# Dane-ME/keypoint-detection

Measured on AMD Instinct MI355X. Metric: images/sec @ 256x192 COCO-17 (MultiPersonKeypointModel.forward, given boxes), higher is better.
Workload: dtype fp32; 1 GPU; C2: batch 64/GPU, 256x192x3, 1 box/img, heatmap head + soft-argmax decode; model=MultiPersonKeypointModel (MobileNetV3-Small+FPN, HeatmapHead), global_batch=64, height=256, width=192, persons=1, precision=split, parallelism=dp1, streams_per_gpu=1, gather=False, gather_pipelined=False

## Files before the change

### include/kpd.h

```cpp
#ifndef KPD_H_
#define KPD_H_

#include <stddef.h>
#include <stdint.h>

#ifdef __cplusplus
extern "C" {
#endif

#define KPD_OK 0
#define KPD_EINVAL (-1)
#define KPD_EHIP (-2)
#define KPD_ESTATE (-3)

#define KPD_PRECISION_FP32 0
#define KPD_PRECISION_MIXED 1
#define KPD_PRECISION_SPLIT 2

typedef struct kpd_plan kpd_plan;

const char* kpd_last_error(void);
const char* kpd_version(void);

int kpd_plan_create(int device, int in_channels, kpd_plan** out);
// ... 115 lines not shown
                              void* stream);

#define KPD_COORD_SMOOTH_L1 0
#define KPD_COORD_MSE 1
#define KPD_COORD_HUBER 2
int kpd_coord_loss(const float* heat, const float* gt, const float* vis, int planes, int H, int W, float temperature,
                   int loss_type, float pixel_weight_scale, float distance_threshold, float* coords, float* loss,
                   float* grad, void* stream);

int kpd_softargmax_backward(const float* heat, const float* grad_coords, int planes, int H, int W, float temperature,
                            float* grad_heat, void* stream);

int kpd_plan_set_streams(kpd_plan* plan, int n);

int kpd_plan_set_graphs(kpd_plan* plan, int enable);

int kpd_bench_conv16(int split, int N, int H, int W, int cin, int cout, int dbg, int iters, float* ms);

#define KPD_BUILD_DIAG 1
int kpd_build_flags(void);

int kpd_fpn0x_class_table(int* cls_ng, int* cls_g, int* cls_woff, int* blocks);


int kpd_heatmap_head(kpd_plan* plan, const float* x, int R, int H, int W, int parts, float* heat, float* ch_w,
                     float* sp_w, void* stream);

int kpd_keypoint_head(kpd_plan* plan, const float* x, int R, int H, int W, float* keypoints, float* visibility,
                      void* stream);

int kpd_backbone(kpd_plan* plan, const float* image, int B, int C, int H, int W, float* out0, float* out1,
                 float* out2, float* out3, void* stream);

int kpd_backbone_body(kpd_plan* plan, const float* image, int B, int C, int H, int W, float* feat0, float* feat1,
                      float* feat2, float* feat3, void* stream);

int kpd_backbone_fpn(kpd_plan* plan, const float* feat0, const float* feat1, const float* feat2, const float* feat3,
                     int B, const int* sizes, float* out0, float* out1, float* out2, float* out3, void* stream);

int kpd_roi_features(kpd_plan* plan, const float* image, int B, int C, int H, int W, const float* boxes, int P,
                     const int32_t* rows, int n, float* out, void* stream);

int kpd_channel_attention(kpd_plan* plan, const float* x, int B, int C, int H, int W, float* scores, int32_t* topk,
                          int k, float* selected, void* stream);

#define KPD_DECODE_ARGMAX 0
// ... 48 lines not shown
```

### keypoint-detection_amd/csrc/conv_glds.hip

```cpp
#include <algorithm>
#include <type_traits>

#include "kpd_common.h"
#include "kpd_kernels.h"
#include "conv_epilogue.h"
#include "kpd_dma.h"

namespace {

typedef _Float16 f16x8 __attribute__((ext_vector_type(8)));
typedef __attribute__((address_space(3))) void lds_void;

constexpr int BM = 256, NT = 512, ROWB = 128;
constexpr unsigned OOB = 0x80000000u;

__device__ __forceinline__ void stamp16(unsigned long long* st, int i, unsigned long long v = 0, int row = -1) {
  if (st && threadIdx.x == 0)
    st[(size_t)(row < 0 ? blockIdx.x : row) * 8 + i] = v ? v : __builtin_amdgcn_s_memrealtime();
}

__device__ __forceinline__ float dpp_xor1(float x) {
  return __int_as_float(__builtin_amdgcn_mov_dpp(__float_as_int(x), 0xB1, 0xF, 0xF, true));
}
__device__ __forceinline__ float dpp_xor2(float x) {
// ... 519 lines not shown
    }
    s_fp[u] = make_int2(x0 | (x1 << 16), y0 | (y1 << 16));
  }
  __syncthreads();
  const int f_tsel = (lchunk >> 1) & 1;
  const unsigned f_byte = (unsigned)((lchunk >> 2) * 32 + (lchunk & 1) * 16);
  const int co_b = wave * (BN / 8) + lrow;

  int cls = 0, n = 0, jt = 0, ca = 0, cb = 0, q0 = 0, NG = 1, NL = 0, KT = 0, ld = 0;
  constexpr int FSH = 22;
  unsigned f_off[A_LD], l_off = 0;
  const float inv_rw = 1.f / (float)rw;
  auto rows = [&](int L, unsigned* fo, unsigned& lo) {
    const int c = L & 15, nj = L >> 4, nn = nj / p.tpc, j = nj - nn * p.tpc;
    const int a_ = c >> 2, b_ = c & 3, qb = j * BM;
    lo = (unsigned)((nn * RG + qb + wave * 32 + lrow) * 512);
#pragma unroll
    for (int i = 0; i < A_LD; ++i) {
      const int q = qb + wave * 32 + i * 8 + lrow;
      const int Y = (int)(((float)q + 0.5f) * inv_rw), X = q - Y * rw, y = 4 * Y + a_, x = 4 * X + b_;
      const unsigned fl = (y > 0 ? 1u : 0u) | (y + 1 < Hf ? 2u : 0u) | (x > 0 ? 4u : 0u) | (x + 1 < Wf ? 8u : 0u) |
                          (Y > 0 ? 16u : 0u) | (Y + 1 < rh ? 32u : 0u) | (X > 0 ? 64u : 0u) |
                          (X + 1 < rw ? 128u : 0u) | (q < RG ? 256u : 0u);
      fo[i] = (unsigned)((nn * Hf + y) * Wf + x) | fl << FSH;
    }
  };
  auto need = [](int dy, int dx, int sh) {
    return ((dy < 0 ? 1u : 0u) | (dy > 0 ? 2u : 0u) | (dx < 0 ? 4u : 0u) | (dx > 0 ? 8u : 0u)) << sh | 256u;
  };
  auto setup = [&](int L) {
    cls = L & 15;
    const int nj = L >> 4;
    n = nj / p.tpc;
    jt = nj - n * p.tpc;
    ca = cls >> 2;
    cb = cls & 3;
    q0 = jt * BM;
    NG = s_ng[cls];
    NL = (kFpn0xSecondMask >> cls) & 1u ? 0 : 4 * NG;
    KT = NL + KT0;
    ld = 0;
  };
  auto issue_tap0 = [&](int stage, int k, const unsigned* fo) {
    const unsigned so = stage * STAGE;
    const int t = 2 * k + f_tsel;
    const int dy = t / 3 - 1, dx = t % 3 - 1;
    const int delta = (dy * Wf + dx) * 64 + (int)f_byte;
    const unsigned nd = t < 9 ? need(dy, dx, 0) : ~0u;
#pragma unroll
    for (int i = 0; i < A_LD; ++i) {
      const unsigned voff = ((fo[i] >> FSH) & nd) == nd ? ((fo[i] << (32 - FSH)) >> (32 - FSH - 6)) + delta : OOB;
      glds16(rf, a_dst + so + i * 8 * ROWB, voff, 0);
    }
#pragma unroll
    for (int i = 0; i < B_LD; ++i)
      glds16(rw0, b_dst + so + i * 8 * ROWB, (unsigned)(((co_b + i * 8) * KT0 + k) * ROWB + lchunk * 16), 0);
  };
  auto issue_at = [&](int stage, int k, int c, int ng, int nl, const unsigned* fo, unsigned lo) {
    const unsigned so = stage * STAGE;
    if (k >= nl) {
      issue_tap0(stage, k - nl, fo);
    } else {
      const int g = k >> 2, kc = k & 3;
      const int gg = s_g[c * 4 + g], oy = gg / 3 - 1, ox = gg % 3 - 1;
      const int delta = (oy * rw + ox) * 512 + kc * 128 + lchunk * 16;
      const unsigned nd = need(oy, ox, 4);
#pragma unroll
      for (int i = 0; i < A_LD; ++i) {
        const unsigned voff = ((fo[i] >> FSH) & nd) == nd ? lo + i * 8 * 512 + delta : OOB;
        glds16(rl, a_dst + so + i * 8 * ROWB, voff, 0);
      }
      const int wbase = s_woff[c] * 2;
#pragma unroll
      for (int i = 0; i < B_LD; ++i)
        glds16(rwe, b_dst + so + i * 8 * ROWB,
               (unsigned)(wbase + (((co_b + i * 8) * ng + g) * 4 + kc) * ROWB + lchunk * 16), 0);
    }
  };
  auto issue = [&](int stage) {
    issue_at(stage, ld, cls, NG, NL, f_off, l_off);
    ++ld;
  };

  f32x4 acc[FM][FN];
// ... 170 lines not shown
        sts[(WAVES_M + wm) * BN + col + r16] = mx;
      }
    }
    __builtin_amdgcn_s_waitcnt(0xC07F);
    __builtin_amdgcn_s_barrier();
    asm volatile("" ::: "memory");
    stamp16(p.stamps, 7, 0, L);
    {
      float v = 0.f;
      if (tid < 2 * BN) {
        const int c = tid & (BN - 1), mxs = tid >= BN;
        v = sts[mxs * WAVES_M * BN + c];
#pragma unroll
        for (int w = 1; w < WAVES_M; ++w) {
          const float u = sts[(mxs * WAVES_M + w) * BN + c];
          v = mxs ? fmaxf(v, u) : v + u;
        }
      }
      const unsigned so = (unsigned)(((e_n * 16 + e_cls) * p.tpc + e_jt) * 2 * BN) * 4u;
      __builtin_amdgcn_raw_buffer_store_b32(__builtin_bit_cast(unsigned, v), rst, tid < 2 * BN ? so + tid * 4 : OOB, 0, 0);
    }
    stamp16(p.stamps, 3, 0, L);
    const int src4 = ((lane & 0x30) | ((lane & 3) << 2) | ((lane >> 2) & 3)) * 4;
    const int2 fp = s_fp[e_n];
    const int fx0 = fp.x & 0xFFFF, fx1 = fp.x >> 16, fy0 = fp.y & 0xFFFF, fy1 = fp.y >> 16;
#pragma unroll
    for (int i = 0; i < FM; ++i)
#pragma unroll
      for (int e = 0; e < 4; ++e) {
        f32x4 v = f32x4{acc[i][0][e], acc[i][1][e], acc[i][2][e], acc[i][3][e]};
        quad_transpose(v, t4);
        f32x4 w;
#pragma unroll
        for (int k = 0; k < 4; ++k) w[k] = __int_as_float(__builtin_amdgcn_ds_bpermute(src4, __float_as_int(v[k])));
        const int q = e_q0 + wm * WM + i * 16 + g * 4 + e;
        const int Y = (int)(((float)q + 0.5f) * inv_rw), X = q - Y * rw;
        const unsigned o =
            (unsigned)((((e_n * Hf + 4 * Y + e_ca) * Wf + 4 * X + e_cb) * BN + wn * 64 + r16 * 4) * 4);
        const int py = 4 * Y + e_ca, px = 4 * X + e_cb;
        const bool keep = q < RG && py >= fy0 && py <= fy1 && px >= fx0 && px <= fx1;
        const unsigned so = keep && (DBG != 4 || (i | e) == 0) ? o : OOB;
        if (p.out_nt) __builtin_amdgcn_raw_buffer_store_b128(__builtin_bit_cast(u32x4, w), rout, so, 0, 2);
        else __builtin_amdgcn_raw_buffer_store_b128(__builtin_bit_cast(u32x4, w), rout, so, 0, 0);
      }
    L = Lnext;
  }
}

// ... 2 lines not shown
                                                         int w_expE, _Float16* __restrict__ out) {
  const int G = cin == 16 ? 16 : 32, c8n = cin / 8;
  const long i = (long)blockIdx.x * blockDim.x + threadIdx.x;
  if (i >= (long)N * hw * c8n) return;
  const long px = i / c8n;
  const int c = (int)(i - px * c8n) * 8, n = (int)(px / hw);
  int a_f, a_l, P;
  fpn0x_exps(sc[(size_t)n * kAmaxStride], sc[(size_t)(N + n) * kAmaxStride], w_exp0, w_expE, &a_f, &a_l, &P);
  const float s = ldexpf(1.f, which ? a_l : a_f);
  const float4 u = *reinterpret_cast<const float4*>(in + px * cin + c);
  const float4 v = *reinterpret_cast<const float4*>(in + px * cin + c + 4);
  const float x[8] = {u.x, u.y, u.z, u.w, v.x, v.y, v.z, v.w};
  typedef _Float16 f16x8v __attribute__((ext_vector_type(8)));
  f16x8v hi, lo;
#pragma unroll
  for (int e = 0; e < 8; ++e) {
    const float xs = x[e] * s;
    hi[e] = (_Float16)xs;
    lo[e] = (_Float16)(xs - (float)hi[e]);
  }
  _Float16* o = out + px * 2 * cin + (c / G) * 2 * G + c % G;
  *reinterpret_cast<f16x8v*>(o) = hi;
  *reinterpret_cast<f16x8v*>(o + G) = lo;
}

constexpr int HP = kHmPitch, HPP = kHmRoiPos;
constexpr int HMS = 56;
constexpr int AWIN = 384;
template <int BMH>
constexpr int hm_awin() { return BMH + 128 <= AWIN ? AWIN : BMH + 128; }
template <int BMH>
constexpr int hm_epi_parts() { return BMH > 256 ? 2 : 1; }
template <int CIN, bool SPLIT>
constexpr int hm_nab() { return (CIN > 0 && (SPLIT ? CIN * 4 : CIN * 2) == 128) ? 1 : 2; }
template <int BMH>
constexpr int kh_epi_parts() { return BMH > 128 ? 2 : 1; }
template <int BN, int BMH>
constexpr int kh_epi_bytes() { return BMH / kh_epi_parts<BMH>() * ((BN + 4) + 68) * 4; }
template <int BN, int SB, int BMH, bool SPLIT, int TPS, int NW, int MODE, int NAB = 2>
constexpr int hmconv_lds_bytes() {
  constexpr int EMODE = MODE >= 0 ? MODE : (BN == 64 ? 1 : 0);
  constexpr int RING = NAB * hm_awin<BMH>() * ROWB + SB * BN * ROWB * TPS;
  constexpr int EPI = EMODE == 2 ? (BN == 128 ? kh_epi_bytes<BN, BMH>() : 0)
                      : EMODE != 0 && EMODE != 3 ? 0 : epi_lds_bytes<BMH / hm_epi_parts<BMH>(), 128, NW * 64>();
  return RING > EPI ? RING : EPI;
}
// ... 1162 lines not shown
  b.stagger = stagger ? 1 : 0;
  static const int out_nt = kpd_diag_env("KPD_FPN0X_NT") ? atoi(kpd_diag_env("KPD_FPN0X_NT")) : 1;
  b.out_nt = out_nt;
  b.spn = spn;
#if KPD_DIAG
  if (dbg == 1) hipLaunchKernelGGL(fpn0x_kernel<1>, dim3((unsigned)grid), dim3(NT), 0, st, b);
  else if (dbg == 2) hipLaunchKernelGGL(fpn0x_kernel<2>, dim3((unsigned)grid), dim3(NT), 0, st, b);
  else if (dbg == 4) hipLaunchKernelGGL(fpn0x_kernel<4>, dim3((unsigned)grid), dim3(NT), 0, st, b);
  else
#endif
  hipLaunchKernelGGL(fpn0x_kernel<0>, dim3((unsigned)grid), dim3(NT), 0, st, b);
  return hipGetLastError();
}

hipError_t launch_split_rows(const float* in, int N, long hw, int cin, const float* sc, int which, int w_exp0,
                             int w_expE, void* out, hipStream_t st) {
  if (cin != 16 && cin % 32 != 0) return hipErrorInvalidValue;
  const long n = (long)N * hw * (cin / 8);
  hipLaunchKernelGGL(split_rows_kernel, dim3((unsigned)((n + 255) / 256)), dim3(256), 0, st, in, N, hw, cin, sc,
                     which, w_exp0, w_expE, static_cast<_Float16*>(out));
  return hipGetLastError();
}

template <int DBG>
static hipError_t bench_launch(const Conv16Args& a, int split, hipStream_t st) {
  if constexpr (DBG == 0) return launch_conv16(a, split, split ? 0 : 1, st);
  dim3 grid(((a.M + BM - 1) / BM) * (a.cout_p / 128));
  if (split) hipLaunchKernelGGL((conv16_kernel<true, float, 3, 128, 3, true, DBG>), grid, dim3(NT), 0, st, a);
  else hipLaunchKernelGGL((conv16_kernel<false, __bf16, 3, 128, 3, true, DBG>), grid, dim3(NT), 0, st, a);
  return hipGetLastError();
}

extern "C" int kpd_bench_conv16(int split, int N, int H, int W, int cin, int cout, int dbg, int iters, float* ms) {
  if (N <= 0 || H <= 0 || W <= 0 || cin % 64 || cout % 128 || iters <= 0 || !ms) return -1;
  if (split && (cin != 128 || cout != 128)) return -1;
  Conv16Args a{};
  const long M = (long)N * H * W;
  const int cin_e = split ? 2 * cin : cin;
  const long in_b = M * cin_e * 2, w_b = (long)cout * 9 * cin_e * 2, out_b = M * cout * 4;
  if (in_b > kMaxDesc) return -1;
  void *in = nullptr, *wt = nullptr, *out = nullptr, *bias = nullptr, *stats = nullptr;
  const bool with_stats = split && ((long)H * W) % BM == 0;
  hipEvent_t e0 = nullptr, e1 = nullptr;
  int rc = -2;
  if (hipMalloc(&in, in_b) != hipSuccess || hipMalloc(&wt, w_b) != hipSuccess || hipMalloc(&out, out_b) != hipSuccess ||
      hipMalloc(&bias, cout * 4) != hipSuccess ||
// ... 44 lines not shown
```

### keypoint-detection_amd/csrc/kpd_common.h

```cpp
#pragma once
#include <hip/hip_runtime.h>
#include <hip/hip_bf16.h>
#include <stdint.h>
#include <stdlib.h>

#ifndef KPD_DIAG
#define KPD_DIAG 0
#endif
static inline const char* kpd_diag_env(const char* name) {
#if KPD_DIAG
  return getenv(name);
#else
  (void)name;
  return nullptr;
#endif
}

typedef float f32x4 __attribute__((ext_vector_type(4)));
typedef __bf16 bf16x8 __attribute__((ext_vector_type(8)));
typedef __bf16 bf16x4 __attribute__((ext_vector_type(4)));
typedef _Float16 f16x4 __attribute__((ext_vector_type(4)));

__device__ __forceinline__ float kpd_div6(float x) {
  constexpr float r6 = 1.f / 6.f;
// ... 40 lines not shown
__device__ __forceinline__ int slot_pos(int s) { return (-1 - s) & 0xFFFF; }
__device__ __forceinline__ bool slot_dummy(int s) { return ((-1 - s) >> 16) & 1; }

__device__ __forceinline__ void amax_publish_img(float* slots, int n, float v) {
  if (v > 0.f) atomicMax(reinterpret_cast<unsigned int*>(slots + (size_t)n * kAmaxStride), __float_as_uint(v));
}

__device__ __forceinline__ int split_exp_of(float amax) {
  const float u = amax * 1.0078125f;
  if (!(u > 0.f)) return 100;
  if (!(u < INFINITY)) return -100;
  int e;
  frexpf(u, &e);
  return min(max(14 - e, -100), 100);
}
__device__ __forceinline__ void fpn0x_exps(float f, float l, int w_exp0, int w_expE, int* a_f, int* a_l, int* P) {
  int pp = min(split_exp_of(f) + w_exp0, split_exp_of(l) + w_expE);
  pp = min(max(pp, -120), 120);
  *P = pp;
  *a_f = pp - w_exp0;
  *a_l = pp - w_expE;
}

#define KPD_CHECK_LAUNCH() (hipGetLastError())
```

### keypoint-detection_amd/csrc/kpd_kernels.h

```cpp
#pragma once
#include <hip/hip_runtime.h>
#include <stdint.h>
#include <vector>

struct ConvArgs {
  const void* in;
  const void* wt;
  const float* bias;
  void* out;
  const float* res;
  const float* a_scale;
  float* stats;
  int N, H, W;
  int cin_p, cout_p;
  int in_cstride, out_cstride;
  int rh, rw;
  int act;
  int M;
  int tiles_per_img;
  float* amax;
  const float* post_scale;
  const float* post_shift;
  int act2, act3;
  int in_bytes, wt_bytes;
// ... 74 lines not shown
  const void* l_split;
  const void* w0;
  const void* weff;
  int cls_woff[16];
  int cls_ng[16];
  int cls_g[16][kFpn0xMaxGroups];
  const float* bias;
  float* out;
  float* stats;
  const float* sc;
  int sc_n;
  int N, Hf, Wf, rh, rw, tpc, w_exp0, w_expE;
  int f_bytes, l_bytes, w0_bytes, weff_bytes;
  int stagger;
  int out_nt;
  int spn;
  unsigned long long* stamps;
  const float* fp_boxes;
  int fp_NB, fp_P;
};
hipError_t launch_fpn0x(const Fpn0xArgs& a, hipStream_t st);
hipError_t launch_split_rows(const float* in, int N, long hw, int cin, const float* sc, int which, int w_exp0,
                             int w_expE, void* out, hipStream_t st);
int conv16_tile_m();

enum ConvDType : int { CONV_F32 = 0, CONV_BF16_OUT_BF16 = 1, CONV_BF16_OUT_F32 = 2 };

int conv_tile_m();
hipError_t launch_conv(const ConvArgs& a, ConvDType dt, int ks, hipStream_t st);

hipError_t launch_stem(const float* img, int N, int Cin, int H, int W, const float* w, const float* b,
                       float* out, int Ho, int Wo, float* amax, hipStream_t st);
hipError_t launch_dwconv(const float* in, const float* w, const float* b, float* out, int N, int H, int W,
                         int Cp, int Ho, int Wo, int k, int s, int act, hipStream_t st);
hipError_t launch_se(const float* x, int N, int HW, int C, int Cp, const float* w1, const float* b1,
                     const float* w2, const float* b2, int sq, float* scale, hipStream_t st,
                     const float* pooled = nullptr);
struct FirArgs {
  const float* x;
  int Hi, Wi, cin_p;
  const float *we, *be;
  const float *wd, *bd;
  const float *wp, *bp;
  int act_e, act_d, Ep, cout_p;
  float* out;
  int Ho, Wo, res;
// ... 265 lines not shown
```

### keypoint-detection_amd/csrc/kpd_pack.hip

```cpp
#include "kpd_plan_int.h"

namespace {

int se_squeeze(int c) {
  const int v = c / 4;
  int n = std::max(8, (int)(v + 4) / 8 * 8);
  if (n < 0.9 * v) n += 8;
  return n;
}

uint16_t f2bf(float f) {
  uint32_t u;
  std::memcpy(&u, &f, 4);
  if ((u & 0x7fffffffu) > 0x7f800000u) return (uint16_t)((u >> 16) | 0x40);
  u += 0x7fffu + ((u >> 16) & 1u);
  return (uint16_t)(u >> 16);
}

const HostT* get(kpd_plan* p, const std::string& name, std::string& missing) {
  auto it = p->t.find(name);
  if (it == p->t.end()) {
    missing += name + " ";
    return nullptr;
  }
// ... 314 lines not shown
                     hE.data() + p->fpn0x.cls_woff[cls]);
  }
  if (int rc = upload(p, h0, &p->fpn0x.w0)) return rc;
  if (int rc = upload(p, hE, &p->fpn0x.weff)) return rc;
  p->fpn0x.w0_bytes = (int)(h0.size() * 2);
  p->fpn0x.weff_bytes = (int)(hE.size() * 2);
  p->fpn0x.w_exp0 = e0;
  p->fpn0x.w_expE = eE;
  return KPD_OK;
}

}

extern "C" {

int kpd_fpn0x_class_table(int* cls_ng, int* cls_g, int* cls_woff, int* blocks) {
  if (!cls_ng || !cls_g || !cls_woff || !blocks) return fail(KPD_EINVAL, "NULL output");
  const int nb = fpn0x_class_table(cls_ng, reinterpret_cast<int(*)[kFpn0xMaxGroups]>(cls_g), cls_woff);
  if (nb < 0) return fail(KPD_ESTATE, "fpn0x: inconsistent class table");
  *blocks = nb;
  return KPD_OK;
}

int kpd_plan_finalize(kpd_plan* p, int precision) {
  if (!p) return fail(KPD_EINVAL, "null plan");
  if (precision != KPD_PRECISION_FP32 && precision != KPD_PRECISION_MIXED && precision != KPD_PRECISION_SPLIT)
    return fail(KPD_EINVAL, "unknown precision");
  HIP_TRY(hipSetDevice(p->device));
  for (void* a : p->allocs) (void)hipFree(a);
  p->allocs.clear();
  p->fpn0x.w0 = p->fpn0x.weff = nullptr;
  p->stamps = nullptr;
  p->pd = DevConv();
  p->anchors = nullptr;
  p->hm1 = DevConv();
  p->hm2 = DevConv();
  p->hm3 = DevConv();
  for (auto& c : p->fpn_lv) c = DevConv();
  p->kh_ds1 = DevConv();
  p->kh_ds2 = DevConv();
  for (auto& k : p->kh_s) k = KhSplit();
  p->kh_split = false;
  p->has_kh = false;
  for (int k = 0; k <= kpd_plan::kMaxSub; ++k) {
    if (p->ws[k]) { (void)hipFree(p->ws[k]); p->ws[k] = nullptr; p->ws_bytes[k] = 0; }
    p->have_work[k] = false;
// ... 213 lines not shown
```

### keypoint-detection_amd/csrc/kpd_plan.hip

```cpp
#include "kpd_plan_int.h"

namespace {
thread_local std::string g_err;
}

int fail(int code, const std::string& msg) {
  g_err = msg;
  return code;
}

int kpd_fail_einval(const char* msg) { return fail(KPD_EINVAL, msg); }
int kpd_fail_hip(hipError_t e, const char* where) {
  return fail(KPD_EHIP, std::string(where) + ": " + hipGetErrorString(e));
}

thread_local KpdPathLog* g_kpd_path = nullptr;

namespace {
struct PathRow { const char* name; unsigned sites; };
const PathRow kPathRows[KP_COUNT] = {
#define KPD_PATH_ROW(id, name, sites) {name, sites},
    KPD_PATH_TOKENS(KPD_PATH_ROW)
#undef KPD_PATH_ROW
};
// ... 775 lines not shown
  lc.c1 = pad16(kFpnIn[1]); lc.c2 = pad16(kFpnIn[2]); lc.c3 = pad16(kFpnIn[3]);
  lc.c1r = kFpnIn[1]; lc.c2r = kFpnIn[2]; lc.c3r = kFpnIn[3];
  lc.S1 = p->lat_S[1]; lc.S2 = p->lat_S[2]; lc.S3 = p->lat_S[3];
  lc.w_exp0 = p->fpn0x.w_exp0; lc.w_expE = p->fpn0x.w_expE;
  lc.h1 = d.h[3]; lc.w1 = d.w[3]; lc.h2 = d.h[8]; lc.w2 = d.w[8]; lc.h3 = d.h[11]; lc.w3 = d.w[11];
  lc.lat1 = w.lat[1];
  lc.lat1_split = ps.lin ? reinterpret_cast<_Float16*>(reinterpret_cast<char*>(w.lat[0]) + (size_t)B * d.h[0] * d.w[0] * 64)
                         : nullptr;
  lc.amax = ps.lin ? w.sc : nullptr;
  static const bool no_chain_t0 = kpd_diag_env("KPD_NO_CHAIN_TAP0") != nullptr;
  if (ps.lin && !no_chain_t0) {
    lc.t0 = taps[0];
    lc.t0_split = reinterpret_cast<_Float16*>(w.lat[0]);
    lc.P0 = d.h[0] * d.w[0];
  }
  lc.stamps = ps.take_stamps("stamps_latchain_0", (size_t)8 * ((B + 7) / 8 * 8));
}

static int lateral0_split_rows(Pass& ps, const float* const taps[4], bool chain, bool chain_t0) {
  kpd_plan* p = ps.p; Work& w = *ps.w; const Dims& d = ps.d;
  char* base = reinterpret_cast<char*>(w.lat[0]);
  if (!chain || !chain_t0) {
    kpd_path(KP_SPLIT_ROWS);
    HIP_TRY(launch_split_rows(taps[0], d.B, (long)d.h[0] * d.w[0], 16, w.sc, 0, p->fpn0x.w_exp0, p->fpn0x.w_expE, base,
                              ps.st));
  }
  if (!chain) {
    kpd_path_at(KP_LAT, 1);
    kpd_path(KP_SPLIT_ROWS);
    HIP_TRY(launch_split_rows(w.lat[1], d.B, (long)d.h[3] * d.w[3], 128, w.sc, 1, p->fpn0x.w_exp0, p->fpn0x.w_expE,
                              base + (size_t)d.B * d.h[0] * d.w[0] * 64, ps.st));
  }
  return KPD_OK;
}

static int stage_laterals(Pass& ps, const float* const taps[4], bool keep_all) {
  kpd_plan* p = ps.p; Work& w = *ps.w; const Dims& d = ps.d;
  const int B = d.B;
  const int lh[4] = {d.h[0], d.h[3], d.h[8], d.h[11]}, lw[4] = {d.w[0], d.w[3], d.w[8], d.w[11]};
  const Stage stage(p, "fpn_lateral", ps.st);
  static const bool no_chain = kpd_diag_env("KPD_NO_LAT_CHAIN") != nullptr;
  LatChainArgs lc{};
  lateral_chain_fill(ps, taps, lc);
  const bool chain = !no_chain && !keep_all && !p->lat[1].bf16 && !p->lat[2].bf16 && !p->lat[3].bf16 &&
                     p->lat[1].cin_p == lc.c1 && p->lat[2].cin_p == lc.c2 && p->lat[3].cin_p == lc.c3 &&
                     p->lat[1].cout_p == 128 && p->lat[2].cout_p == 128 && p->lat[3].cout_p == 128 &&
                     lateral_chain_ok(lc);
  kpd_path(chain ? KP_LAT_CHAIN : KP_LAT_PER_LEVEL);
// ... 65 lines not shown
}

static int stage_topk(Pass& ps, const FwdArgs& a) {
  kpd_plan* p = ps.p; Work& w = *ps.w; const Dims& d = ps.d;
  const int B = d.B, HWf = d.Hf * d.Wf;
  const Stage stage(p, "topk", ps.st);
  if (!d.fused_stats) {
    kpd_path(KP_CHANNEL_STATS);
    HIP_TRY(launch_channel_stats(w.feat, B, HWf, 128, d.tiles, w.stats, ps.st));
  }
  const bool slot_in_topk = a.slot_in_topk();
  if (slot_in_topk) kpd_path(KP_TOPK_SLOTMAP);
  HIP_TRY(launch_topk(w.stats, B, d.tiles, HWf, p->ca_w0, p->ca_b0, p->ca_w2, p->ca_b2, w.topk, w.scores, ps.st,
                      slot_in_topk ? a.boxes : nullptr, a.P, slot_in_topk ? w.slot : nullptr, w.imax,
                      ps.lin ? w.sc : nullptr, B));
  if (ps.lin) w.sc_dirty = false;
  return KPD_OK;
}

static int publish_backbone(Pass& ps, const FwdArgs& a, const float* const taps[4]) {
  Work& w = *ps.w; const Dims& d = ps.d;
  const size_t B = d.B;
  if (a.topk_out) HIP_TRY(hipMemcpyAsync(a.topk_out, w.topk, sizeof(int32_t) * B * 64, hipMemcpyDeviceToDevice, ps.st));
  if (!level0_footprint(ps, a)) ps.dbg["feat0"] = {w.feat, sizeof(float) * B * d.Hf * d.Wf * 128};
  ps.dbg["scores"] = {w.scores, sizeof(float) * B * 128};
  ps.dbg["tap0"] = {taps[0], sizeof(float) * B * d.h[0] * d.w[0] * 16};
  ps.dbg["tap1"] = {taps[1], sizeof(float) * B * d.h[3] * d.w[3] * pad16(24)};
  ps.dbg["tap2"] = {taps[2], sizeof(float) * B * d.h[8] * d.w[8] * pad16(48)};
  ps.dbg["tap3"] = {taps[3], sizeof(float) * B * d.h[11] * d.w[11] * 576};
  if (ps.debug) ps.p->debug = ps.dbg;
  return KPD_OK;
}

static int stage_detect(Pass& ps, const FwdArgs& a) {
  kpd_plan* p = ps.p; Work& w = *ps.w; const Dims& d = ps.d;
  const int B = d.B;
  const Stage sg(p, "person_detect", ps.st);
  static const bool pd_unfused = kpd_diag_env("KPD_PD_UNFUSED") != nullptr;
  if (!pd_unfused && p->pd.cin == 128 && p->pd.cin_p == 128 && p->pd.cout_p == 48 && !p->pd.bf16 &&
      person_detect_fits(d.Wf)) {
    kpd_path(KP_PD_FUSED);
    HIP_TRY(launch_person_detect(w.feat, B, d.Hf, d.Wf, static_cast<const float*>(p->pd.w), p->pd.b, p->anchors, a.H,
                                 a.W, p->det_conf, w.pd_boxes, w.pd_scores, ps.st));
  } else {
    kpd_path(KP_PD_UNFUSED);
    HIP_TRY(launch_adaptive_pool56(w.feat, B, d.Hf, d.Wf, 128, w.pd_pool, ps.st));
    kpd_path_at(KP_PD);
// ... 707 lines not shown
```

### keypoint-detection_amd/csrc/lateral_chain.hip

```cpp
#include <algorithm>

#include "kpd_common.h"
#include "kpd_kernels.h"

namespace {

constexpr int LG = 16;

__device__ __forceinline__ int up_index(int y, int H, int h) {
  return H == h ? y : min((int)floorf((float)y * ((float)h / (float)H)), h - 1);
}

__device__ __forceinline__ void stamp(unsigned long long* st, int i) {
  if (st && threadIdx.x == 0)
    st[((size_t)blockIdx.y * gridDim.x + blockIdx.x) * 8 + i] = __builtin_amdgcn_s_memrealtime();
}

__device__ __forceinline__ f32x4 mfma_k16(const float4 a, const float4 b, f32x4 acc) {
  acc = __builtin_amdgcn_mfma_f32_16x16x4f32(a.x, b.x, acc, 0, 0, 0);
  acc = __builtin_amdgcn_mfma_f32_16x16x4f32(a.y, b.y, acc, 0, 0, 0);
  acc = __builtin_amdgcn_mfma_f32_16x16x4f32(a.z, b.z, acc, 0, 0, 0);
  return __builtin_amdgcn_mfma_f32_16x16x4f32(a.w, b.w, acc, 0, 0, 0);
}

// ... 186 lines not shown
          const int y = pp / p.w1, x = pp - y * p.w1;
          const int sy = up_index(y, p.h1, p.h2), sx = up_index(x, p.w1, p.w2);
          const float v = acc[e] + l2[(sy * p.w2 + sx) * LG + r16];
          if constexpr (SPLIT) {
            const float xs = v * s_l;
            const _Float16 hi = (_Float16)xs;
            tsc[(4 * g + e) * 32 + r16] = hi;
            tsc[(4 * g + e) * 32 + 16 + r16] = (_Float16)(xs - (float)hi);
          } else {
            out[(size_t)pp * 128] = v;
          }
        }
        if constexpr (SPLIT) {
          const int q = lane >> 2, pp = t * 16 + q;
          const uint4 v = *reinterpret_cast<const uint4*>(tsc + q * 32 + part * 8);
          if (pp < P1) *reinterpret_cast<uint4*>(outs + (size_t)pp * 256) = v;
        }
      }
    }
  }
  stamp(p.stamps, 4);
  if constexpr (SPLIT) {
    if (p.t0) {
      const int P0 = p.P0, n8 = P0 * 2, per = (n8 + 7) / 8, i0 = cg * per, i1 = min(i0 + per, n8);
      const float* src = p.t0 + (size_t)b * P0 * 16;
      _Float16* dst = p.t0_split + (size_t)b * P0 * 32;
      typedef _Float16 f16x8v __attribute__((ext_vector_type(8)));
      for (int j0 = i0 + tid; j0 < i1; j0 += 4 * NW * 64) {
        float4 u[4][2];
#pragma unroll
        for (int v = 0; v < 4; ++v) {
          const int j = min(j0 + v * NW * 64, i1 - 1), px = j >> 1, c = (j & 1) * 8;
          u[v][0] = *reinterpret_cast<const float4*>(src + (size_t)px * 16 + c);
          u[v][1] = *reinterpret_cast<const float4*>(src + (size_t)px * 16 + c + 4);
        }
#pragma unroll
        for (int v = 0; v < 4; ++v) {
          const int j = j0 + v * NW * 64, px = j >> 1, c = (j & 1) * 8;
          if (j >= i1) continue;
          const float x[8] = {u[v][0].x, u[v][0].y, u[v][0].z, u[v][0].w, u[v][1].x, u[v][1].y, u[v][1].z, u[v][1].w};
          f16x8v hi, lo;
#pragma unroll
          for (int e = 0; e < 8; ++e) {
            const float xs = x[e] * s_f;
            hi[e] = (_Float16)xs;
            lo[e] = (_Float16)(xs - (float)hi[e]);
          }
          _Float16* o = dst + (size_t)px * 32 + c;
          *reinterpret_cast<f16x8v*>(o) = hi;
          *reinterpret_cast<f16x8v*>(o + 16) = lo;
        }
      }
    }
  }
  stamp(p.stamps, 5);
}

}

size_t lateral_chain_lds_bytes(const LatChainArgs& a) {
  const size_t P2 = (size_t)a.h2 * a.w2, P3 = (size_t)a.h3 * a.w3;
  return (P3 * LG + std::max(P2, NW * P3) * LG + 4 * NW) * sizeof(float) + (size_t)NW * 16 * 2 * LG * 2;
}

bool lateral_chain_ok(const LatChainArgs& a) {
  return a.c1 == 32 && a.c2 == 48 && a.c3 == 576 && a.h1 > 0 && a.w1 > 0 && a.h2 > 0 && a.w2 > 0 && a.h3 > 0 &&
         a.w3 > 0 && a.h3 * a.w3 <= 16 * 8 && lateral_chain_lds_bytes(a) <= 80 * 1024 &&
         (!a.lat1_split || a.amax);
}

hipError_t launch_lateral_chain(const LatChainArgs& a, int B, hipStream_t st) {
  if (B <= 0) return hipSuccess;
  if (!lateral_chain_ok(a)) return hipErrorInvalidValue;
  LatChainArgs q = a;
  q.n = B;
  const dim3 grid((unsigned)((B + 7) / 8 * 8), 128 / LG), block(NW * 64);
  const size_t lds = lateral_chain_lds_bytes(a);
  const bool small = a.h3 * a.w3 <= 16 * 3;
  static const bool noreuse = kpd_diag_env("KPD_LC_NOREUSE") != nullptr;
  const bool reuse = !noreuse && (long)a.h1 * a.w1 <= 6 * NW * 16;
  if (a.lat1_split && small && reuse) {
    kpd_path(KP_LC_SPLIT_SMALL_REUSE);
    hipLaunchKernelGGL((lateral_chain_kernel<2, 3, 36, 3, 6, true, true>), grid, block, lds, st, q);
  } else if (a.lat1_split && reuse) {
    kpd_path(KP_LC_SPLIT_BIG_REUSE);
    hipLaunchKernelGGL((lateral_chain_kernel<2, 3, 36, 8, 6, true, true>), grid, block, lds, st, q);
  } else if (a.lat1_split) {
    kpd_path(small ? KP_LC_SPLIT_SMALL : KP_LC_SPLIT_BIG);
    if (small) hipLaunchKernelGGL((lateral_chain_kernel<2, 3, 36, 3, 6, true>), grid, block, lds, st, q);
    else hipLaunchKernelGGL((lateral_chain_kernel<2, 3, 36, 8, 6, true>), grid, block, lds, st, q);
  } else {
// ... 7 lines not shown
```

### keypoint-detection_amd/dll/_native.py

```python
from __future__ import annotations

import ctypes
import os
from pathlib import Path
from typing import List, Optional

import torch

_LIB_PATH = Path(__file__).resolve().parent / "_lib" / "libkpd.so"
_lib: Optional[ctypes.CDLL] = None

KPD_PRECISION_FP32 = 0
KPD_PRECISION_MIXED = 1
KPD_PRECISION_SPLIT = 2
PRECISIONS = {"fp32": KPD_PRECISION_FP32, "split": KPD_PRECISION_SPLIT, "mixed": KPD_PRECISION_MIXED,
              "bf16": KPD_PRECISION_MIXED}

EXPORTS = ("kpd_last_error", "kpd_version", "kpd_plan_create", "kpd_plan_set_tensor",
           "kpd_plan_finalize", "kpd_plan_destroy", "kpd_forward", "kpd_debug_copy", "kpd_nms",
           "kpd_plan_timing", "kpd_plan_timing_stage", "kpd_plan_timing_query", "kpd_plan_set_detector",
           "kpd_bench_conv16", "kpd_build_flags", "kpd_fpn0x_class_table",
           "kpd_plan_set_streams", "kpd_preprocess", "kpd_target_heatmaps", "kpd_keypoint_metrics",
           "kpd_heatmap_head", "kpd_keypoint_head", "kpd_backbone", "kpd_channel_attention", "kpd_decode_heatmaps",
           "kpd_roi_align", "kpd_conv1x1", "kpd_adaptive_heatmap_loss", "kpd_conv3x3_forward",
           "kpd_conv3x3_backward", "kpd_conv3x3_forward_prec", "kpd_conv3x3_backward_prec", "kpd_plan_set_graphs", "kpd_backbone_body", "kpd_backbone_fpn",
           "kpd_plan_path_log", "kpd_plan_path_query", "kpd_preprocess_batch", "kpd_draw_poses",
           "kpd_oks_match", "kpd_pose_nms", "kpd_flip_merge", "kpd_augment_batch", "kpd_bn_train_forward",
           "kpd_bn_train_backward", "kpd_roi_targets", "kpd_roi_features", "kpd_detector_features",
           "kpd_detector_targets", "kpd_detector_loss", "kpd_coord_loss", "kpd_softargmax_backward")
PRE_BATCH_CHUNK = 32
DRAW_BOXES, DRAW_LIMBS, DRAW_JOINTS, DRAW_HEAT = 1, 2, 4, 8
DRAW_CHUNK = 32
DRAW_TILE_W = 64
DRAW_TILE_H = 16
DRAW_MAX_SIDE = 16384
DRAW_MAX_WIDTH = 512
DRAW_MAX_HEAT = 1024
OKS_MAX_K = 32
OKS_MAX_T = 16
OKS_MAX_D = 64
OKS_MAX_G = 64
POSE_NMS_MAX_D = 64
POSE_NMS_MAX_K = 32
POSE_NMS_HARD, POSE_NMS_SOFT, POSE_NMS_SOFT_LINEAR = 0, 1, 2
# ... 60 lines not shown
    lib.kpd_plan_path_query.argtypes = [c_void_p, c_char_p, ctypes.c_size_t, ctypes.POINTER(ctypes.c_size_t)]
    lib.kpd_target_heatmaps.argtypes = [c_void_p, c_int, c_int, c_int, ctypes.c_double, c_void_p, c_void_p]
    lib.kpd_keypoint_metrics.argtypes = [c_void_p, c_void_p, c_void_p, ctypes.c_long, ctypes.POINTER(ctypes.c_float),
                                         c_int, c_void_p, c_void_p]
    lib.kpd_preprocess_batch.argtypes = [ctypes.POINTER(c_void_p), ctypes.POINTER(c_int), ctypes.POINTER(c_int),
                                         ctypes.POINTER(c_int), c_int, c_int, c_int, ctypes.c_float, c_int, c_int,
                                         c_int, c_int, ctypes.POINTER(ctypes.c_float),
                                         ctypes.POINTER(ctypes.c_float), c_void_p, c_void_p]
    u8p = ctypes.POINTER(ctypes.c_uint8)
    lib.kpd_draw_poses.argtypes = [ctypes.POINTER(c_void_p), ctypes.POINTER(c_int), ctypes.POINTER(c_int),
                                   ctypes.POINTER(c_int), c_int, c_void_p, c_void_p, c_void_p, c_void_p,
                                   c_int, c_int, c_int, c_int, ctypes.POINTER(c_int), c_int, u8p, u8p, u8p,
                                   c_int, c_int, c_int, c_int, c_int, c_int, c_int, c_void_p]
    lib.kpd_oks_match.argtypes = [c_void_p] * 8 + [ctypes.POINTER(ctypes.c_float)] * 2 + [c_int] * 6 + \
        [c_void_p] * 8
    lib.kpd_pose_nms.argtypes = [c_void_p] * 5 + [ctypes.POINTER(ctypes.c_float)] + [c_int] * 4 + \
        [ctypes.c_float] * 3 + [c_int] + [c_void_p] * 6
    lib.kpd_flip_merge.argtypes = [c_void_p] * 3 + [ctypes.POINTER(ctypes.c_int32)] + [c_int] * 5 + [c_void_p] * 5
    i32p = ctypes.POINTER(ctypes.c_int32)
    lib.kpd_augment_batch.argtypes = [ctypes.POINTER(c_void_p)] + [ctypes.POINTER(c_int)] * 3 + \
        [ctypes.POINTER(c_void_p), c_int, c_int, i32p, ctypes.POINTER(ctypes.c_double), ctypes.POINTER(c_int),
         i32p, i32p, u8p, i32p, c_void_p, c_void_p, c_void_p, c_int, c_int, c_void_p, c_void_p, c_void_p, c_void_p]
    lib.kpd_fpn0x_class_table.argtypes = [ctypes.POINTER(c_int)] * 4
    lib.kpd_nms.argtypes = [c_void_p, c_void_p, c_int, ctypes.c_float, c_int, c_void_p, c_void_p, c_void_p]
    c_float = ctypes.c_float
    lib.kpd_heatmap_head.argtypes = [c_void_p, c_void_p, c_int, c_int, c_int, c_int, c_void_p, c_void_p, c_void_p,
                                     c_void_p]
    lib.kpd_keypoint_head.argtypes = [c_void_p, c_void_p, c_int, c_int, c_int, c_void_p, c_void_p, c_void_p]
    lib.kpd_backbone.argtypes = [c_void_p, c_void_p, c_int, c_int, c_int, c_int, c_void_p, c_void_p, c_void_p,
                                 c_void_p, c_void_p]
    lib.kpd_backbone_body.argtypes = [c_void_p, c_void_p, c_int, c_int, c_int, c_int, c_void_p, c_void_p, c_void_p,
                                      c_void_p, c_void_p]
    lib.kpd_backbone_fpn.argtypes = [c_void_p, c_void_p, c_void_p, c_void_p, c_void_p, c_int,
                                     ctypes.POINTER(c_int), c_void_p, c_void_p, c_void_p, c_void_p, c_void_p]
    lib.kpd_channel_attention.argtypes = [c_void_p, c_void_p, c_int, c_int, c_int, c_int, c_void_p, c_void_p, c_int,
                                          c_void_p, c_void_p]
    lib.kpd_decode_heatmaps.argtypes = [c_void_p, c_int, c_int, c_int, c_int, c_float, c_void_p, c_void_p, c_void_p,
                                        c_void_p]
    lib.kpd_roi_align.argtypes = [c_void_p, c_int, c_int, c_int, c_int, c_void_p, c_int, c_int, c_int, c_float, c_int,
                                  c_int, c_void_p, c_void_p]
    lib.kpd_conv1x1.argtypes = [c_void_p, c_int, c_int, c_int, c_void_p, c_void_p, c_int, c_void_p, c_void_p]
    lib.kpd_adaptive_heatmap_loss.argtypes = [c_void_p, c_void_p, c_void_p, c_int, c_int, c_int, c_int, c_float,
                                              c_float, c_int, c_float, c_void_p, c_void_p, c_void_p, c_void_p]
    lib.kpd_conv3x3_forward.argtypes = [c_void_p, c_void_p, c_void_p, c_int, c_int, c_int, c_int, c_int, c_void_p,
                                        c_void_p]
    lib.kpd_conv3x3_backward.argtypes = [c_void_p, c_void_p, c_void_p, c_int, c_int, c_int, c_int, c_int, c_void_p,
# ... 638 lines not shown
```

Before: 41350 images/s.

## Store split tap0 in stride-4 phase planes and skip stores outside footprint

Reorders the split fp16 hi/lo tap0 buffer feeding the fpn0x kernel from plain row-major pixels into 16 phase planes (one per y&3, x&3 class), each laid out on the coarse grid. The goal is contiguous per-class gathers for tap0 loads. The split kernel and the lateral-chain split path now write this layout, and the conv address math is adjusted to match. The conv epilogue also checks whether a wave's output rows intersect the box footprint and, if not, issues out-of-bounds no-op stores instead of computing outputs. This adds index arithmetic and depends on P0 == 16*h1*w1.

```diff
diff --git a/include/kpd.h b/include/kpd.h
--- a/include/kpd.h
+++ b/include/kpd.h
@@ -161,6 +161,8 @@
 
 int kpd_fpn0x_class_table(int* cls_ng, int* cls_g, int* cls_woff, int* blocks);
 
+int kpd_fpn0x_plane_rows(int N, int Hf, int Wf, int* rows);
+
 
 int kpd_heatmap_head(kpd_plan* plan, const float* x, int R, int H, int W, int parts, float* heat, float* ch_w,
                      float* sp_w, void* stream);
diff --git a/keypoint-detection_amd/csrc/conv_glds.hip b/keypoint-detection_amd/csrc/conv_glds.hip
--- a/keypoint-detection_amd/csrc/conv_glds.hip
+++ b/keypoint-detection_amd/csrc/conv_glds.hip
@@ -565,7 +565,7 @@
       const unsigned fl = (y > 0 ? 1u : 0u) | (y + 1 < Hf ? 2u : 0u) | (x > 0 ? 4u : 0u) | (x + 1 < Wf ? 8u : 0u) |
                           (Y > 0 ? 16u : 0u) | (Y + 1 < rh ? 32u : 0u) | (X > 0 ? 64u : 0u) |
                           (X + 1 < rw ? 128u : 0u) | (q < RG ? 256u : 0u);
-      fo[i] = (unsigned)((nn * Hf + y) * Wf + x) | fl << FSH;
+      fo[i] = (unsigned)((nn * 16 + c) * RG + q) | fl << FSH;
     }
   };
   auto need = [](int dy, int dx, int sh) {
@@ -584,11 +584,12 @@
     KT = NL + KT0;
     ld = 0;
   };
-  auto issue_tap0 = [&](int stage, int k, const unsigned* fo) {
+  auto issue_tap0 = [&](int stage, int k, int c, const unsigned* fo) {
     const unsigned so = stage * STAGE;
     const int t = 2 * k + f_tsel;
     const int dy = t / 3 - 1, dx = t % 3 - 1;
-    const int delta = (dy * Wf + dx) * 64 + (int)f_byte;
+    const int ay = (c >> 2) + dy, bx = (c & 3) + dx;
+    const int delta = ((((ay & 3) * 4 + (bx & 3)) - c) * RG + (ay >> 2) * rw + (bx >> 2)) * 64 + (int)f_byte;
     const unsigned nd = t < 9 ? need(dy, dx, 0) : ~0u;
 #pragma unroll
     for (int i = 0; i < A_LD; ++i) {
@@ -602,7 +603,7 @@
   auto issue_at = [&](int stage, int k, int c, int ng, int nl, const unsigned* fo, unsigned lo) {
     const unsigned so = stage * STAGE;
     if (k >= nl) {
-      issue_tap0(stage, k - nl, fo);
+      issue_tap0(stage, k - nl, c, fo);
     } else {
       const int g = k >> 2, kc = k & 3;
       const int gg = s_g[c * 4 + g], oy = gg / 3 - 1, ox = gg % 3 - 1;
@@ -819,8 +820,19 @@
     }
     stamp16(p.stamps, 3, 0, L);
     const int src4 = ((lane & 0x30) | ((lane & 3) << 2) | ((lane >> 2) & 3)) * 4;
-    const int2 fp = s_fp[e_n];
+    const int2 fpv = s_fp[e_n];
+    const int2 fp = make_int2(__builtin_amdgcn_readfirstlane(fpv.x), __builtin_amdgcn_readfirstlane(fpv.y));
     const int fx0 = fp.x & 0xFFFF, fx1 = fp.x >> 16, fy0 = fp.y & 0xFFFF, fy1 = fp.y >> 16;
+    bool any_keep;
+    {
+      const int qa = __builtin_amdgcn_readfirstlane(e_q0 + wm * WM), qb = min(qa + WM, RG) - 1;
+      const int ry0 = (fy0 - e_ca + 3) >> 2, ry1 = (fy1 - e_ca) >> 2, rx0 = (fx0 - e_cb + 3) >> 2, rx1 = (fx1 - e_cb) >> 2;
+      any_keep = max(qa, ry0 * rw) <= min(qb, ry1 * rw + rw - 1) && max(rx0, 0) <= min(rx1, rw - 1);
+    }
+    if (__builtin_amdgcn_readfirstlane(any_keep ? 1 : 0) == 0) {
+#pragma unroll
+      for (int i = 0; i < FM * 4; ++i) __builtin_amdgcn_raw_buffer_store_b32((unsigned)src4, rout, OOB, 0, 0);
+    } else
 #pragma unroll
     for (int i = 0; i < FM; ++i)
 #pragma unroll
@@ -869,6 +881,37 @@
   _Float16* o = out + px * 2 * cin + (c / G) * 2 * G + c % G;
   *reinterpret_cast<f16x8v*>(o) = hi;
   *reinterpret_cast<f16x8v*>(o + G) = lo;
+}
+
+__global__ __launch_bounds__(256) void split_tap0_planes_kernel(const float* __restrict__ in, int N, int rh, int rw,
+                                                                const float* __restrict__ sc, int w_exp0, int w_expE,
+                                                                _Float16* __restrict__ out) {
+  const int Hf = 4 * rh, Wf = 4 * rw, units = Hf * ((rw + 7) >> 3);
+  const long i = (long)blockIdx.x * blockDim.x + threadIdx.x;
+  const int n = (int)(i / ((long)units * 64));
+  if (n >= N) return;
+  const int r = (int)(i - (long)n * units * 64);
+  int y, x, c;
+  fpn0x_plane_item(r >> 6, r & 63, rw, &y, &x, &c);
+  if (x < 0) return;
+  int a_f, a_l, P;
+  fpn0x_exps(sc[(size_t)n * kAmaxStride], sc[(size_t)(N + n) * kAmaxStride], w_exp0, w_expE, &a_f, &a_l, &P);
+  const float s = ldexpf(1.f, a_f);
+  const float* src = in + ((size_t)(n * Hf + y) * Wf + x) * 16 + c;
+  const float4 u = *reinterpret_cast<const float4*>(src);
+  const float4 v = *reinterpret_cast<const float4*>(src + 4);
+  const float xv[8] = {u.x, u.y, u.z, u.w, v.x, v.y, v.z, v.w};
+  typedef _Float16 f16x8v __attribute__((ext_vector_type(8)));
+  f16x8v hi, lo;
+#pragma unroll
+  for (int e = 0; e < 8; ++e) {
+    const float xs = xv[e] * s;
+    hi[e] = (_Float16)xs;
+    lo[e] = (_Float16)(xs - (float)hi[e]);
+  }
+  _Float16* o = out + (size_t)fpn0x_plane_row(n, y, x, rw, rh * rw) * 32 + c;
+  *reinterpret_cast<f16x8v*>(o) = hi;
+  *reinterpret_cast<f16x8v*>(o + 16) = lo;
 }
 
 constexpr int HP = kHmPitch, HPP = kHmRoiPos;
@@ -2077,6 +2120,15 @@
   return hipGetLastError();
 }
 
+hipError_t launch_split_tap0_planes(const float* in, int N, int rh, int rw, const float* sc, int w_exp0, int w_expE,
+                                    void* out, hipStream_t st) {
+  if (N <= 0 || rh <= 0 || rw <= 0) return hipErrorInvalidValue;
+  const long n = (long)N * 4 * rh * ((rw + 7) / 8) * 64;
+  hipLaunchKernelGGL(split_tap0_planes_kernel, dim3((unsigned)((n + 255) / 256)), dim3(256), 0, st, in, N, rh, rw, sc,
+                     w_exp0, w_expE, static_cast<_Float16*>(out));
+  return hipGetLastError();
+}
+
 template <int DBG>
 static hipError_t bench_launch(const Conv16Args& a, int split, hipStream_t st) {
   if constexpr (DBG == 0) return launch_conv16(a, split, split ? 0 : 1, st);
diff --git a/keypoint-detection_amd/csrc/kpd_common.h b/keypoint-detection_amd/csrc/kpd_common.h
--- a/keypoint-detection_amd/csrc/kpd_common.h
+++ b/keypoint-detection_amd/csrc/kpd_common.h
@@ -86,4 +86,14 @@
   *a_l = pp - w_expE;
 }
 
+__host__ __device__ __forceinline__ int fpn0x_plane_row(int n, int y, int x, int rw, int RG) {
+  return (n * 16 + (y & 3) * 4 + (x & 3)) * RG + (y >> 2) * rw + (x >> 2);
+}
+__host__ __device__ __forceinline__ void fpn0x_plane_item(int unit, int it, int rw, int* y, int* x, int* c) {
+  const int nxc = (rw + 7) >> 3, xc = unit % nxc, pi = it >> 1, X = xc * 8 + (pi & 7);
+  *y = unit / nxc;
+  *x = X < rw ? 4 * X + (pi >> 3) : -1;
+  *c = (it & 1) * 8;
+}
+
 #define KPD_CHECK_LAUNCH() (hipGetLastError())
diff --git a/keypoint-detection_amd/csrc/kpd_kernels.h b/keypoint-detection_amd/csrc/kpd_kernels.h
--- a/keypoint-detection_amd/csrc/kpd_kernels.h
+++ b/keypoint-detection_amd/csrc/kpd_kernels.h
@@ -120,6 +120,8 @@
 hipError_t launch_fpn0x(const Fpn0xArgs& a, hipStream_t st);
 hipError_t launch_split_rows(const float* in, int N, long hw, int cin, const float* sc, int which, int w_exp0,
                              int w_expE, void* out, hipStream_t st);
+hipError_t launch_split_tap0_planes(const float* in, int N, int rh, int rw, const float* sc, int w_exp0, int w_expE,
+                                    void* out, hipStream_t st);
 int conv16_tile_m();
 
 enum ConvDType : int { CONV_F32 = 0, CONV_BF16_OUT_BF16 = 1, CONV_BF16_OUT_F32 = 2 };
diff --git a/keypoint-detection_amd/csrc/kpd_pack.hip b/keypoint-detection_amd/csrc/kpd_pack.hip
--- a/keypoint-detection_amd/csrc/kpd_pack.hip
+++ b/keypoint-detection_amd/csrc/kpd_pack.hip
@@ -360,6 +360,17 @@
   return KPD_OK;
 }
 
+int kpd_fpn0x_plane_rows(int N, int Hf, int Wf, int* rows) {
+  if (!rows) return fail(KPD_EINVAL, "NULL output");
+  if (N <= 0 || Hf <= 0 || Wf <= 0 || Hf % 4 || Wf % 4 || (long)N * Hf * Wf >= (1L << 31))
+    return fail(KPD_EINVAL, "fpn0x planes: N > 0 and Hf, Wf positive multiples of 4");
+  const int rh = Hf / 4, rw = Wf / 4;
+  for (int n = 0; n < N; ++n)
+    for (int y = 0; y < Hf; ++y)
+      for (int x = 0; x < Wf; ++x) rows[((size_t)n * Hf + y) * Wf + x] = fpn0x_plane_row(n, y, x, rw, rh * rw);
+  return KPD_OK;
+}
+
 int kpd_plan_finalize(kpd_plan* p, int precision) {
   if (!p) return fail(KPD_EINVAL, "null plan");
   if (precision != KPD_PRECISION_FP32 && precision != KPD_PRECISION_MIXED && precision != KPD_PRECISION_SPLIT)
diff --git a/keypoint-detection_amd/csrc/kpd_plan.hip b/keypoint-detection_amd/csrc/kpd_plan.hip
--- a/keypoint-detection_amd/csrc/kpd_plan.hip
+++ b/keypoint-detection_amd/csrc/kpd_plan.hip
@@ -821,8 +821,8 @@
   char* base = reinterpret_cast<char*>(w.lat[0]);
   if (!chain || !chain_t0) {
     kpd_path(KP_SPLIT_ROWS);
-    HIP_TRY(launch_split_rows(taps[0], d.B, (long)d.h[0] * d.w[0], 16, w.sc, 0, p->fpn0x.w_exp0, p->fpn0x.w_expE, base,
-                              ps.st));
+    HIP_TRY(launch_split_tap0_planes(taps[0], d.B, d.h[3], d.w[3], w.sc, p->fpn0x.w_exp0, p->fpn0x.w_expE, base,
+                                     ps.st));
   }
   if (!chain) {
     kpd_path_at(KP_LAT, 1);
@@ -934,7 +934,7 @@
   Work& w = *ps.w; const Dims& d = ps.d;
   const size_t B = d.B;
   if (a.topk_out) HIP_TRY(hipMemcpyAsync(a.topk_out, w.topk, sizeof(int32_t) * B * 64, hipMemcpyDeviceToDevice, ps.st));
-  if (!level0_footprint(ps, a)) ps.dbg["feat0"] = {w.feat, sizeof(float) * B * d.Hf * d.Wf * 128};
+  ps.dbg[level0_footprint(ps, a) ? "feat0_footprint" : "feat0"] = {w.feat, sizeof(float) * B * d.Hf * d.Wf * 128};
   ps.dbg["scores"] = {w.scores, sizeof(float) * B * 128};
   ps.dbg["tap0"] = {taps[0], sizeof(float) * B * d.h[0] * d.w[0] * 16};
   ps.dbg["tap1"] = {taps[1], sizeof(float) * B * d.h[3] * d.w[3] * pad16(24)};
diff --git a/keypoint-detection_amd/csrc/lateral_chain.hip b/keypoint-detection_amd/csrc/lateral_chain.hip
--- a/keypoint-detection_amd/csrc/lateral_chain.hip
+++ b/keypoint-detection_amd/csrc/lateral_chain.hip
@@ -232,7 +232,8 @@
   stamp(p.stamps, 4);
   if constexpr (SPLIT) {
     if (p.t0) {
-      const int P0 = p.P0, n8 = P0 * 2, per = (n8 + 7) / 8, i0 = cg * per, i1 = min(i0 + per, n8);
+      const int P0 = p.P0, RG = p.h1 * p.w1, Wf = 4 * p.w1, units = 4 * p.h1 * ((p.w1 + 7) >> 3);
+      const int n8 = units * 64, per = (units + 7) / 8 * 64, i0 = cg * per, i1 = min(i0 + per, n8);
       const float* src = p.t0 + (size_t)b * P0 * 16;
       _Float16* dst = p.t0_split + (size_t)b * P0 * 32;
       typedef _Float16 f16x8v __attribute__((ext_vector_type(8)));
@@ -240,14 +241,21 @@
         float4 u[4][2];
 #pragma unroll
         for (int v = 0; v < 4; ++v) {
-          const int j = min(j0 + v * NW * 64, i1 - 1), px = j >> 1, c = (j & 1) * 8;
+          const int j = min(j0 + v * NW * 64, i1 - 1);
+          int y, x, c;
+          fpn0x_plane_item(j >> 6, j & 63, p.w1, &y, &x, &c);
+          const int px = y * Wf + max(x, 0);
           u[v][0] = *reinterpret_cast<const float4*>(src + (size_t)px * 16 + c);
           u[v][1] = *reinterpret_cast<const float4*>(src + (size_t)px * 16 + c + 4);
         }
 #pragma unroll
         for (int v = 0; v < 4; ++v) {
-          const int j = j0 + v * NW * 64, px = j >> 1, c = (j & 1) * 8;
+          const int j = j0 + v * NW * 64;
           if (j >= i1) continue;
+          int y, xp, c;
+          fpn0x_plane_item(j >> 6, j & 63, p.w1, &y, &xp, &c);
+          if (xp < 0) continue;
+          const int px = fpn0x_plane_row(0, y, xp, p.w1, RG);
           const float x[8] = {u[v][0].x, u[v][0].y, u[v][0].z, u[v][0].w, u[v][1].x, u[v][1].y, u[v][1].z, u[v][1].w};
           f16x8v hi, lo;
 #pragma unroll
@@ -276,7 +284,7 @@
 bool lateral_chain_ok(const LatChainArgs& a) {
   return a.c1 == 32 && a.c2 == 48 && a.c3 == 576 && a.h1 > 0 && a.w1 > 0 && a.h2 > 0 && a.w2 > 0 && a.h3 > 0 &&
          a.w3 > 0 && a.h3 * a.w3 <= 16 * 8 && lateral_chain_lds_bytes(a) <= 80 * 1024 &&
-         (!a.lat1_split || a.amax);
+         (!a.lat1_split || a.amax) && (!a.t0 || a.P0 == 16 * a.h1 * a.w1);
 }
 
 hipError_t launch_lateral_chain(const LatChainArgs& a, int B, hipStream_t st) {
diff --git a/keypoint-detection_amd/dll/_native.py b/keypoint-detection_amd/dll/_native.py
--- a/keypoint-detection_amd/dll/_native.py
+++ b/keypoint-detection_amd/dll/_native.py
@@ -19,7 +19,7 @@
 EXPORTS = ("kpd_last_error", "kpd_version", "kpd_plan_create", "kpd_plan_set_tensor",
            "kpd_plan_finalize", "kpd_plan_destroy", "kpd_forward", "kpd_debug_copy", "kpd_nms",
            "kpd_plan_timing", "kpd_plan_timing_stage", "kpd_plan_timing_query", "kpd_plan_set_detector",
-           "kpd_bench_conv16", "kpd_build_flags", "kpd_fpn0x_class_table",
+           "kpd_bench_conv16", "kpd_build_flags", "kpd_fpn0x_class_table", "kpd_fpn0x_plane_rows",
            "kpd_plan_set_streams", "kpd_preprocess", "kpd_target_heatmaps", "kpd_keypoint_metrics",
            "kpd_heatmap_head", "kpd_keypoint_head", "kpd_backbone", "kpd_channel_attention", "kpd_decode_heatmaps",
            "kpd_roi_align", "kpd_conv1x1", "kpd_adaptive_heatmap_loss", "kpd_conv3x3_forward",
@@ -126,6 +126,7 @@
         [ctypes.POINTER(c_void_p), c_int, c_int, i32p, ctypes.POINTER(ctypes.c_double), ctypes.POINTER(c_int),
          i32p, i32p, u8p, i32p, c_void_p, c_void_p, c_void_p, c_int, c_int, c_void_p, c_void_p, c_void_p, c_void_p]
     lib.kpd_fpn0x_class_table.argtypes = [ctypes.POINTER(c_int)] * 4
+    lib.kpd_fpn0x_plane_rows.argtypes = [c_int, c_int, c_int, ctypes.POINTER(c_int)]
     lib.kpd_nms.argtypes = [c_void_p, c_void_p, c_int, ctypes.c_float, c_int, c_void_p, c_void_p, c_void_p]
     c_float = ctypes.c_float
     lib.kpd_heatmap_head.argtypes = [c_void_p, c_void_p, c_int, c_int, c_int, c_int, c_void_p, c_void_p, c_void_p,
```

Result: no change. 41440 images/s, median of 6 (+0.2%).
